# hadimsnj/SGRACEx1

Hardware: AMD Instinct MI355X
Metric: edges aggregated/sec, 2-layer GCN forward (higher is better)
Workload: dtype f16 (f32 accumulate); 1 GPU; s100m; nodes_per_gpu=4194304, edges_per_gpu=104193983, generator=uniform, f_in=1433, hidden=64, layer1=gemm_mode=0 sparse X, relu=1, layer2=gemm_mode=1 dense X, relu=0, exchange=none

## Files before the change

include/sgx.h:

```cpp
#ifndef SGX_H
#define SGX_H

#include <stddef.h>
#include <stdint.h>

#ifdef __cplusplus
extern "C" {
#endif

#define SGX_VERSION 110

typedef enum sgx_status {
    SGX_OK = 0,
    SGX_ERR_NULL = -1,
    SGX_ERR_SHAPE = -2,
    SGX_ERR_UNSUPPORTED = -3,
    SGX_ERR_WORKSPACE = -4,
    SGX_ERR_HIP = -5,
    SGX_ERR_CSR = -6,
    SGX_ERR_ALIGN = -7,
    SGX_ERR_SEEDS = -8,
    SGX_ERR_BLOCKS = -9
} sgx_status;

typedef enum sgx_dtype { SGX_F16 = 0, SGX_F32 = 1 } sgx_dtype;

typedef enum sgx_acc_mode { SGX_ACC_F32 = 0, SGX_ACC_REF_HALF = 1 } sgx_acc_mode;

typedef struct sgx_plan sgx_plan;

int sgx_plan_create(sgx_plan **plan, const int32_t *rowPtr, int n_rows, int n_feat_hint,
                    void *stream);
int sgx_plan_create_ex(sgx_plan **plan, const int32_t *rowPtr, int n_rows, int long_threshold, int chunk,
                       void *stream);
void sgx_plan_destroy(sgx_plan *plan);
int sgx_plan_long_rows(const sgx_plan *plan);
int sgx_plan_long_threshold(const sgx_plan *plan);
float sgx_plan_natural_utilization(const sgx_plan *plan);
int sgx_plan_reordered(const sgx_plan *plan);
int64_t sgx_plan_export(const sgx_plan *plan, int which, int32_t *dst, int64_t capacity, void *stream);
int sgx_xw_sparse_form(int dtype, int n_rows, int M_fea, int P, const void *W, int64_t ldw, const void *H, int64_t ldh,
                       const sgx_plan *plan);

#define SGX_QUANT_ADJ_DONE 1
#define SGX_QUANT_INT8 2
#define SGX_QUANT_INT8_AUTO 4
typedef struct sgx_quant {
    int32_t qbits;
    int32_t scale_fea;
    int32_t internal_bits;
    int32_t flags;
    float   inv_scale_fea;
    float   zero_fea;
    float   inv_scale_w;
    float   zero_w;
    float   inv_scale_adj;
    float   zero_adj;
    float   deq_factor;
    float   reserved;
    int64_t nnz_adj;
    int64_t nnz_fea;
} sgx_quant;

int sgx_fake_quantize(int is_signed, int qbits, float inv_scale, float zero, int64_t n, const float *x,
                      float *out, void *stream);
// ... 659 lines not shown
```

sgracex1_amd/csrc/layer.hip:

```cpp
#include "sgx_internal.h"

namespace {

struct Carve {
    size_t h_off, h_bytes;
    size_t w_off, w_bytes;
    size_t s_off, s_bytes;
    size_t g_off, g_bytes;
    size_t q_off, q_bytes;
    size_t qb, qx, qa, qt;
    size_t qw;
    int64_t ldc;
    size_t total;
};

bool repitch_x(const sgx_layer_desc *d)
{
    return sgx_ldh(d->dtype, d->M_fea) != d->M_fea && (int64_t)d->M_adj * d->M_fea >= (int64_t)1 << 22;
}

bool int8_form(const sgx_layer_desc *d)
{
    if (!d->quant || d->gemm_mode != 1 || d->quant->qbits > 8 || d->P_w > 256) return false;
    if (d->quant->flags & SGX_QUANT_INT8) return true;
// ... 194 lines not shown
        ep_d.out_scale = q->deq_factor;
    }

    int scores_ready = 0;
    if (d->gat_mode && !q && d->gemm_mode == 1 && d->acc_mode == SGX_ACC_F32 && attention &&
        sgx_gat_scores_fusable(d->dtype, d->P_w, d->gat_heads, d->plan_adj)) {
        const int heads = d->gat_heads < 1 ? 1 : d->gat_heads;
        float *gs = (float *)(ws + c.g_off);
        const sgx_gat_scratch lay = sgx_gat_scratch_layout(d->M_adj, d->P_w, heads, d->gat_fill_dead_rows, d->plan_adj);
        const bool direct = d->P_w / heads == 32;
        float *s1 = gs + (direct ? lay.s1 : lay.sp1), *s2 = gs + (direct ? lay.s2 : lay.sp2);
        rc = (direct || lay.has_partials)
                 ? sgx_xw_dense_scores(d->M_adj, d->M_fea, d->P_w, values_fea, d->M_fea, B, d->M_fea, H, ldh, attention, heads, s1, s2, s)
                 : SGX_ERR_UNSUPPORTED;
        if (rc == SGX_OK && !direct) rc = sgx_gat_scores_combine(gs, lay, d->M_adj, d->P_w, heads, s);
        if (rc == SGX_OK) scores_ready = 1;
        else if (rc != SGX_ERR_UNSUPPORTED) return rc;
    }
    if (scores_ready) {
        rc = SGX_OK;
    } else if (c.ldc) {
        rc = sgx_xw_dense_i8(q->qbits, d->M_adj, d->M_fea, d->P_w, (const int8_t *)values_fea, c.ldc, (const int8_t *)B, c.ldc,
                             q->scale_fea, q->internal_bits, (float *)H, ldh, ws + c.q_off + c.qw, s);
    } else if (d->gemm_mode == 0) {
        rc = sgx_transpose(d->dtype, d->P_w, d->M_fea, B, d->M_fea, W, ldh, s);
        if (rc != SGX_OK) return rc;
        rc = sgx_spmm_launch(d->dtype, d->acc_mode, d->spmm_block, 0, d->M_adj, d->M_fea, d->P_w, d->rowPtr_fea,
                             d->columnIndex_fea, values_fea, W, ldh, H, ldh, d->plan_fea, scratch, c.s_bytes, s, nullptr,
                             nullptr, 0, true, thread_count(d->fea_threads), ep_h);
    } else if (d->acc_mode == SGX_ACC_REF_HALF && thread_count(d->fea_threads) > 1) {
        if (d->dtype != SGX_F16) return SGX_ERR_UNSUPPORTED;
        if (ldh > d->P_w) SGX_HIP_CHECK(hipMemsetAsync(H, 0, (size_t)d->M_adj * ldh * sizeof(f16), s));
        rc = sgx_refhalf_dense(d->spmm_block, d->fea_threads, d->M_adj, d->M_fea, d->P_w, values_fea, d->M_fea, B, d->M_fea,
                               H, ldh, s);
    } else {
        rc = sgx_xw_dense_ep(d->dtype, d->acc_mode, d->spmm_block, d->M_adj, d->M_fea, d->P_w, values_fea, d->M_fea, B, d->M_fea,
                             H, ldh, s, ep_h);
    }
    if (rc != SGX_OK) return rc;

    if (d->ev_agg_begin) SGX_HIP_CHECK(hipEventRecord((hipEvent_t)d->ev_agg_begin, s));
    if (d->gat_mode) {
        if (!attention) return SGX_ERR_NULL;
        rc = sgx_gat_aggregate_ep(d->dtype, d->relu, d->gat_fill_dead_rows, d->N_adj, d->M_adj, d->P_w, d->gat_heads, d->alpha,
                                  d->rowPtr_adj, d->columnIndex_adj,
                                  values_adj, H, ldh, attention, d->D, d->P_w, (float *)d->E, (float *)d->S, d->plan_adj,
// ... 79 lines not shown
```

sgracex1_amd/csrc/sgx_internal.h:

```cpp
#pragma once
#include <hip/hip_runtime.h>
#include <stdint.h>
#include <stddef.h>

#include <atomic>
#include <type_traits>

#include "sgx.h"

#define SGX_HIP_CHECK(expr)                     \
    do {                                        \
        hipError_t _e = (expr);                 \
        if (_e != hipSuccess) return SGX_ERR_HIP; \
    } while (0)

#define SGX_LAUNCH_CHECK()                                   \
    do {                                                     \
        if (hipGetLastError() != hipSuccess) return SGX_ERR_HIP; \
    } while (0)

typedef _Float16 f16;

struct sgx_lds_optin {
    static constexpr int kDevices = 64;
    std::atomic<bool> done[kDevices];
};
template <typename Kernel>
int sgx_raise_dynamic_lds(Kernel kernel, sgx_lds_optin &optin, size_t bytes)
{
    int dev = 0;
    SGX_HIP_CHECK(hipGetDevice(&dev));
    const bool known = dev >= 0 && dev < sgx_lds_optin::kDevices;
    if (known && optin.done[dev].load(std::memory_order_acquire)) return SGX_OK;
    SGX_HIP_CHECK(hipFuncSetAttribute(reinterpret_cast<const void *>(kernel), hipFuncAttributeMaxDynamicSharedMemorySize, (int)bytes));
    if (known) optin.done[dev].store(true, std::memory_order_release);
    return SGX_OK;
}

struct sgx_tuning {
    bool gat_one_pass, gat_no_fused_scores;
    int gat_fused;
    int gat_scan;
    bool xw_no_wlds, xw_no_stationary_f32, xw_sparse_no_lds, xw_short_tiles, xw_no_lds;
    bool xtg_scalar, xtg_wave_tiles;
    bool spmm_no_short_tail;
    bool layer_no_fused_dense;
    int spmm_fused_blocks_per_cu;
    int spmm_cpl;
    int xw_sparse_lpr;
    int xw_sparse_streams;
    int plan_long_threshold;
    int plan_chunk;
    float plan_reorder_below;
};
const sgx_tuning &sgx_tune();

static inline size_t sgx_elem_size(int dtype) { return dtype == SGX_F16 ? 2 : 4; }
static inline size_t sgx_align_up(size_t x, size_t a) { return (x + a - 1) / a * a; }
static inline int sgx_next_pow2(int x) { int p = 1; while (p < x) p <<= 1; return p; }

struct sgx_plan {
    int n_rows;
    int64_t nnz;
    int long_threshold;
    int chunk;
    int n_long;
    int n_tasks;
    int32_t *long_row;
    int32_t *long_first;
    int32_t *task_row;
// ... 38 lines not shown
}

int sgx_refhalf_csr(int spmm_block, int threads, int relu, int n_rows, int n_cols, int n_feat, const int32_t *rowPtr, const int32_t *columnIndex,
                    const void *values, const void *table, int64_t ldt, void *out, int64_t ldo, hipStream_t s);
int sgx_refhalf_dense(int spmm_block, int threads, int n_rows, int M, int n_feat, const void *X, int64_t ldx, const void *Wt,
                      int64_t ldw, void *out, int64_t ldo, hipStream_t s);

int sgx_spmm_launch(int dtype, int acc_mode, int spmm_block, int relu, int n_rows, int n_cols, int n_feat,
                    const int32_t *rowPtr, const int32_t *columnIndex, const void *values,
                    const void *H, int64_t ldh, void *D, int64_t ldd,
                    const sgx_plan *plan, void *scratch, size_t scratch_bytes, hipStream_t stream,
                    const float *acc_in = nullptr, float *acc_out = nullptr, int64_t ld_acc = 0,
                    bool fea_stage = false, int ref_threads = 1, sgx_epilogue ep = sgx_no_epilogue());

bool sgx_spmm_table_big(int dtype, int n_cols, int64_t ldh, int n_feat);

bool sgx_spmm_dense_applicable(int n_cols, const void *X, const void *Wt, const void *D, const sgx_plan *plan);
int sgx_spmm_dense(int relu, int n_rows, int n_cols, const int32_t *rowPtr, const int32_t *columnIndex, const void *values,
                   const void *X, const void *Wt, void *D, hipStream_t stream);

bool sgx_xw_sparse_lds_applicable(int dtype, int n_rows, int m_fea, int n_feat, int64_t ldh, const sgx_plan *plan);
int sgx_xw_sparse_lds(int dtype, int n_rows, int m_fea, int n_feat, const int32_t *rowPtr, const int32_t *columnIndex,
                      const void *values, const void *W, int64_t ldw, void *H, int64_t ldh, const sgx_plan *plan,
                      sgx_epilogue ep, hipStream_t stream);

int sgx_repitch_rows(const void *src, int64_t src_pitch, void *dst, int64_t dst_pitch, int row_bytes, int64_t n_rows,
                     hipStream_t stream);
struct sgx_xw_form {
    int kind, a, b, blocks, vec, wgs_per_cu;
    int64_t waves;
};
bool sgx_xw_dense_wlds_form(int n_rows, int M, int P, const void *X, int64_t ldx, const void *Wt, int64_t ldw, const void *H,
                            int64_t ldh, sgx_xw_form *form);
bool sgx_xw_dense_wlds_f32_form(int n_rows, int M, int P, const void *Wt, int64_t ldw, const void *H, int64_t ldh, int h_aligned,
                                sgx_xw_form *form);
int sgx_xw_dense_wlds(int n_rows, int M, int P, const void *X, int64_t ldx, const void *Wt, int64_t ldw, void *H, int64_t ldh,
                      int relu, hipStream_t stream);
int sgx_xw_dense_wlds_f32(int n_rows, int M, int P, const void *X, int64_t ldx, const void *Wt, int64_t ldw, void *H, int64_t ldh,
                          int h_aligned, sgx_epilogue ep, int relu, hipStream_t stream);
int sgx_xw_dense_ep(int dtype, int acc_mode, int spmm_block, int n_rows, int M_fea, int P, const void *X, int64_t ldx,
                    const void *Wt, int64_t ldw, void *H, int64_t ldh, hipStream_t stream, sgx_epilogue ep, int relu = 0);
int sgx_gat_aggregate_ep(int dtype, int relu, int fill_dead_rows, int n_rows, int n_cols, int n_feat, int n_heads, float alpha,
                         const int32_t *rowPtr, const int32_t *columnIndex, const void *values, const void *Wh, int64_t ldh,
                         const void *attention, void *D, int64_t ldd, float *E, float *S, const sgx_plan *plan,
                         float *s_scratch, hipStream_t stream, float out_scale, const float *ext_fill = nullptr, int ext_n = 0,
                         int scores_ready = 0);

// ... 88 lines not shown
```

sgracex1_amd/csrc/spmm_csr.hip:

```cpp
#include "sgx_device.h"

#ifndef SGX_SPMM_MINWAVES
#define SGX_SPMM_MINWAVES 1
#endif
#ifndef SGX_SPMM_NT_STORE
#define SGX_SPMM_NT_STORE 0
#endif
#include <stdlib.h>

#ifndef SGX_SPMM_ADJ_STYLE
#define SGX_SPMM_ADJ_STYLE 0
#endif
#ifndef SGX_SPMM_FEA_STYLE
#define SGX_SPMM_FEA_STYLE 1
#endif
#ifndef SGX_SPMM_PIECES
#define SGX_SPMM_PIECES 1
#endif
#ifndef SGX_SPMM_BLOCKS_PER_CU
#define SGX_SPMM_BLOCKS_PER_CU 512
#endif

namespace {

// ... 295 lines not shown

template <typename T, int VEC, int LPR, int CPL, bool BIG>
__global__ __launch_bounds__(kBlock, SGX_SPMM_MINWAVES) void spmm_short_tail_kernel(SGX_SPMM_PARAMS)
{
    spmm_body<T, VEC, LPR, CPL, BIG, SGX_SPMM_ADJ_STYLE, true>(SGX_SPMM_ARGS);
}

template <typename T, int VEC, int LPR, int CPL, bool BIG>
__global__ __launch_bounds__(kBlock, SGX_SPMM_MINWAVES) void xw_sparse_kernel(SGX_SPMM_PARAMS)
{
    spmm_body<T, VEC, LPR, CPL, BIG, SGX_SPMM_FEA_STYLE, false>(SGX_SPMM_ARGS);
}

typedef _Float16 f16x8 __attribute__((ext_vector_type(8)));
typedef f16x8 f16x8_u __attribute__((aligned(2)));
typedef float f32x4 __attribute__((ext_vector_type(4)));

constexpr int kDenseF = 64;
constexpr int kDenseTile = 16;
constexpr int kDensePitch = kDenseF + 8;
#ifndef SGX_SPMM_DENSE_BLOCKS_PER_CU
#define SGX_SPMM_DENSE_BLOCKS_PER_CU 256
#endif

__device__ __forceinline__ void wave_lds_sync()
{
    __builtin_amdgcn_fence(__ATOMIC_RELEASE, "wavefront");
    __builtin_amdgcn_wave_barrier();
    __builtin_amdgcn_fence(__ATOMIC_ACQUIRE, "wavefront");
}

__global__ __launch_bounds__(kBlock, SGX_SPMM_MINWAVES) void spmm_dense_f16_kernel(
    int n_rows, const int32_t *__restrict__ rowptr, const int32_t *__restrict__ col, const f16 *__restrict__ val,
    const f16 *__restrict__ X, unsigned x_bytes, const f16 *__restrict__ Wt, f16 *__restrict__ D, int relu)
{
    constexpr int VEC = 8, LPR = 8, RPW = 64 / LPR, KS = kDenseF / 32, NT = kDenseF / 16;
    __shared__ __attribute__((aligned(16))) f16x8 sW[KS][NT][64];
    __shared__ __attribute__((aligned(16))) f16 sZ[kBlock / 64][kDenseTile * kDensePitch];
    const int lane = threadIdx.x & 63;
    const int sub = lane % LPR, grp = lane / LPR;
    const int l15 = lane & 15, lq = lane >> 4;

    for (int i = threadIdx.x; i < KS * NT * 64; i += kBlock) {
        const int ln = i & 63, nt = (i >> 6) % NT, s = i / (64 * NT);
        const int n = (nt / 2) * 32 + 8 * ((ln & 15) / 4) + 4 * (nt % 2) + (ln & 15) % 4;
        sW[s][nt][ln] = *reinterpret_cast<const f16x8_u *>(Wt + n * kDenseF + s * 32 + 8 * (ln >> 4));
    }
    __syncthreads();

    const __amdgpu_buffer_rsrc_t rsrc = __builtin_amdgcn_make_buffer_rsrc(const_cast<f16 *>(X), 0, x_bytes, 0x00020000);
    const unsigned chunk_off[1] = {(unsigned)(sub * VEC) * (unsigned)sizeof(f16)};
    f16 *slab = sZ[threadIdx.x >> 6];
// ... 28 lines not shown
#pragma unroll
            for (int nt = 0; nt < NT; ++nt) d[nt] = __builtin_amdgcn_mfma_f32_16x16x32_f16(sW[s][nt][lane], b, d[nt], 0, 0, 0);
        }
        wave_lds_sync();
#pragma unroll
        for (int q = 0; q < NT / 2; ++q) {
            f16x8 o;
#pragma unroll
            for (int j = 0; j < 4; ++j) {
                const f16 lo = (f16)d[2 * q][j], hi = (f16)d[2 * q + 1][j];
                o[j] = (!relu || lo > (f16)0) ? lo : (f16)0;
                o[4 + j] = (!relu || hi > (f16)0) ? hi : (f16)0;
            }
            *reinterpret_cast<f16x8 *>(slab + l15 * kDensePitch + q * 32 + 8 * lq) = o;
        }
        wave_lds_sync();
#pragma unroll
        for (int h = 0; h < kDenseTile / RPW; ++h) {
            const int64_t r = r0 + h * RPW + grp;
            const u32x4 v = *reinterpret_cast<const u32x4 *>(slab + (h * RPW + grp) * kDensePitch + sub * VEC);
            if (r < n_rows) *reinterpret_cast<Elem<f16>::vec16_u *>(D + r * kDenseF + sub * VEC) = v;
        }
        wave_lds_sync();
    }
}

template <typename T>
__global__ __launch_bounds__(kBlock) void spmm_split_finalize_kernel(
    int n_long, int n_feat, const int32_t *__restrict__ long_row, const int32_t *__restrict__ long_first,
    const float *__restrict__ partial, int ldp, T *__restrict__ D, int64_t ldd, int relu,
    const float *__restrict__ acc_in, float *__restrict__ acc_out, int64_t ld_acc, sgx_epilogue ep)
{
    const int64_t gid = (int64_t)blockIdx.x * kBlock + threadIdx.x;
    const int64_t total = (int64_t)n_long * n_feat;
    if (gid >= total) return;
    const int l = (int)(gid / n_feat), j = (int)(gid % n_feat);
    const int64_t row = long_row[l];
    float s = acc_in ? acc_in[row * ld_acc + j] : 0.0f;
    const int t_end = long_first[l + 1];
    int t = long_first[l];
    for (; t + 8 <= t_end; t += 8) {
        float v[8];
#pragma unroll
        for (int u = 0; u < 8; ++u) v[u] = partial[(int64_t)(t + u) * ldp + j];
#pragma unroll
        for (int u = 0; u < 8; ++u) s += v[u];
// ... 117 lines not shown
}

bool sgx_spmm_table_big(int dtype, int n_cols, int64_t ldh, int n_feat)
{
    const size_t es = sgx_elem_size(dtype);
    return (unsigned long long)n_cols * (unsigned long long)ldh * es > kOOBRow || (unsigned long long)n_feat * es > kMaxRowBytes;
}

bool sgx_spmm_dense_applicable(int n_cols, const void *X, const void *Wt, const void *D, const sgx_plan *plan)
{
    if (plan && (plan->n_tasks > 0 || plan->row_order)) return false;
    if (sgx_spmm_table_big(SGX_F16, n_cols, kDenseF, kDenseF)) return false;
    return (uintptr_t)X % 4 == 0 && (uintptr_t)Wt % 2 == 0 && (uintptr_t)D % 2 == 0;
}

int sgx_spmm_dense(int relu, int n_rows, int n_cols, const int32_t *rowPtr, const int32_t *columnIndex, const void *values,
                   const void *X, const void *Wt, void *D, hipStream_t stream)
{
    if (n_rows < 0 || n_cols < 0) return SGX_ERR_SHAPE;
    if (n_rows == 0) return SGX_OK;
    if (!rowPtr || !Wt || !D) return SGX_ERR_NULL;
    if (n_cols > 0 && (!X || !columnIndex || !values)) return SGX_ERR_NULL;
    if (!sgx_spmm_dense_applicable(n_cols, X, Wt, D, nullptr)) return SGX_ERR_UNSUPPORTED;
    const int64_t rows_per_block = (int64_t)kDenseTile * (kBlock / 64);
    int64_t blocks = ((int64_t)n_rows + rows_per_block - 1) / rows_per_block;
    const int per_cu = sgx_tune().spmm_fused_blocks_per_cu > 0 ? sgx_tune().spmm_fused_blocks_per_cu : SGX_SPMM_DENSE_BLOCKS_PER_CU;
    if (blocks > (int64_t)256 * per_cu) blocks = (int64_t)256 * per_cu;
    hipLaunchKernelGGL(spmm_dense_f16_kernel, dim3((unsigned)blocks), dim3(kBlock), 0, stream, n_rows, rowPtr, columnIndex,
                       (const f16 *)values, (const f16 *)X, (unsigned)((size_t)n_cols * kDenseF * sizeof(f16)), (const f16 *)Wt,
                       (f16 *)D, relu);
    SGX_LAUNCH_CHECK();
    return SGX_OK;
}

int sgx_spmm_launch(int dtype, int acc_mode, int spmm_block, int relu, int n_rows, int n_cols, int n_feat,
                    const int32_t *rowPtr, const int32_t *columnIndex, const void *values,
                    const void *H, int64_t ldh, void *D, int64_t ldd,
                    const sgx_plan *plan, void *scratch, size_t scratch_bytes, hipStream_t stream,
                    const float *acc_in, float *acc_out, int64_t ld_acc, bool fea_stage, int ref_threads, sgx_epilogue ep)
{
    (void)spmm_block;
    if (n_rows < 0 || n_cols < 0 || n_feat < 1 || ldh < n_feat) return SGX_ERR_SHAPE;
    if (n_rows == 0) return SGX_OK;
    if (!rowPtr || (!D && !acc_out)) return SGX_ERR_NULL;
    if (D && ldd < n_feat) return SGX_ERR_SHAPE;
    if ((acc_in || acc_out) && (ld_acc < n_feat || acc_mode != SGX_ACC_F32)) return SGX_ERR_SHAPE;
    if (dtype != SGX_F16 && dtype != SGX_F32) return SGX_ERR_UNSUPPORTED;
    if (acc_mode == SGX_ACC_REF_HALF) {
        if (dtype != SGX_F16) return SGX_ERR_UNSUPPORTED;
        if (n_cols > 0 && (!H || !columnIndex || !values)) return SGX_ERR_NULL;
        return sgx_refhalf_csr(spmm_block, ref_threads, relu, n_rows, n_cols, n_feat, rowPtr, columnIndex, values, H, ldh, D, ldd, stream);
    }
    if (acc_mode != SGX_ACC_F32) return SGX_ERR_UNSUPPORTED;
    if (plan && plan->n_rows != n_rows) return SGX_ERR_SHAPE;
    const size_t es = sgx_elem_size(dtype);
// ... 54 lines not shown
```

sgracex1_amd/csrc/util_kernels.hip:

```cpp
#include "sgx_internal.h"

#include <stdlib.h>

namespace {

constexpr int kBlock = 256;

template <typename T>
__global__ __launch_bounds__(kBlock) void transpose_kernel(int rows, int cols, const T *__restrict__ in, int64_t ldi,
                                                           T *__restrict__ out, int64_t ldo)
{
    __shared__ T tile[32][33];
    const int tx = threadIdx.x & 31, ty = threadIdx.x >> 5;
    const int r0 = blockIdx.y * 32, c0 = blockIdx.x * 32;
    for (int i = ty; i < 32; i += 8) {
        const int r = r0 + i, c = c0 + tx;
        tile[i][tx] = (r < rows && c < cols) ? in[(int64_t)r * ldi + c] : (T)0;
    }
    __syncthreads();
    for (int i = ty; i < 32; i += 8) {
        const int c = c0 + i, r = r0 + tx;
        if (c < cols && r < ldo) out[(int64_t)c * ldo + r] = (r < rows) ? tile[tx][i] : (T)0;
    }
}
// ... 237 lines not shown

namespace {
sgx_tuning g_tuning;
bool g_tuning_loaded = false;
void load_tuning()
{
    sgx_tuning t{};
    auto flag = [](const char *name) { return getenv(name) != nullptr; };
    auto num = [](const char *name) { const char *v = getenv(name); return v ? atoi(v) : 0; };
    t.gat_one_pass = flag("SGX_GAT_ONE_PASS");
    t.gat_no_fused_scores = flag("SGX_GAT_NO_FUSED_SCORES");
    { const char *v = getenv("SGX_GAT_SCAN"); t.gat_scan = v ? atoi(v) : 1; }
    { const char *v = getenv("SGX_GAT_FUSED"); t.gat_fused = v ? atoi(v) : 1; }
    t.xw_no_wlds = flag("SGX_XW_NO_WLDS");
    t.xw_no_stationary_f32 = flag("SGX_XW_NO_STATIONARY_F32");
    t.xw_sparse_no_lds = flag("SGX_XW_SPARSE_NO_LDS");
    t.xw_short_tiles = flag("SGX_XW_SHORT_TILES");
    t.xw_no_lds = flag("SGX_XW_NO_LDS");
    t.xtg_scalar = flag("SGX_XTG_SCALAR");
    t.xtg_wave_tiles = flag("SGX_XTG_WAVE_TILES");
    t.spmm_no_short_tail = flag("SGX_SPMM_NO_SHORT_TAIL");
    t.layer_no_fused_dense = flag("SGX_LAYER_NO_FUSED_DENSE");
    t.spmm_fused_blocks_per_cu = num("SGX_SPMM_FUSED_BLOCKS_PER_CU");
    t.spmm_cpl = num("SGX_SPMM_CPL");
    t.xw_sparse_lpr = num("SGX_XW_SPARSE_LPR");
    t.xw_sparse_streams = num("SGX_XW_SPARSE_STREAMS");
    t.plan_long_threshold = num("SGX_PLAN_LONG_THRESHOLD");
    t.plan_chunk = num("SGX_PLAN_CHUNK");
    const char *rb = getenv("SGX_PLAN_REORDER_BELOW");
    t.plan_reorder_below = rb ? (float)atof(rb) : -1.0f;
    g_tuning = t;
    g_tuning_loaded = true;
}
}

const sgx_tuning &sgx_tune()
{
    if (!g_tuning_loaded) load_tuning();
    return g_tuning;
}

extern "C" void sgx_reload_env(void) { load_tuning(); }
```

sgracex1_amd/csrc/xw_sparse_lds.hip:

```cpp
#include "sgx_device.h"

#include <stdlib.h>
#include <type_traits>

namespace {

constexpr int kWaves = 16;
constexpr int kThreads = kWaves * 64;
#ifndef SGX_XW_LDS_DEPTH
#define SGX_XW_LDS_DEPTH 8
#endif
#ifndef SGX_XW_LDS_SKIP_UNUSED
#define SGX_XW_LDS_SKIP_UNUSED 1
#endif
#ifndef SGX_XW_LDS_PAIRS
#define SGX_XW_LDS_PAIRS 0
#endif
constexpr unsigned kFarOOB = 0xFFFF0000u;
constexpr int kDepth = SGX_XW_LDS_DEPTH;
constexpr size_t kLdsBudget = 160 * 1024;

template <int EPS, int TT> __device__ __forceinline__ unsigned step_bcast(unsigned x)
{
    if constexpr (EPS == 1) return x;
    else if constexpr (EPS == 4)
        return (unsigned)__builtin_amdgcn_mov_dpp((int)x, TT | (TT << 2) | (TT << 4) | (TT << 6), 0xF, 0xF, true);
    else
        return (unsigned)__builtin_amdgcn_mov_dpp((int)x, TT | (TT << 2) | ((2 + TT) << 4) | ((2 + TT) << 6), 0xF, 0xF, true);
}

template <typename T, int VEC, int LPR, bool FULL>
__global__ __launch_bounds__(kThreads) void xw_sparse_lds_kernel(
    int n_rows, int n_feat, int m_fea, const int32_t *__restrict__ rowptr, const int32_t *__restrict__ col,
    const T *__restrict__ val, const T *__restrict__ W, int64_t ldw, int w_vec, T *__restrict__ H, int64_t ldh,
    int n_split, unsigned nnz_bytes_col, const uint8_t *__restrict__ win_order, sgx_epilogue ep)
{
    extern __shared__ __attribute__((aligned(16))) unsigned char lds[];
    constexpr int CP = LPR * VEC;
    constexpr unsigned ROWB = LPR * 16;
    constexpr int RPW = 64 / LPR;
    constexpr int SUBS = LPR;
    constexpr int EPS = LPR >= 4 ? 4 : LPR;
    constexpr int D = kDepth;

    const int xcd = blockIdx.x & 7, q = blockIdx.x >> 3;
    const int streams_per_xcd = (int)(gridDim.x >> 3) / n_split;
    if (q >= streams_per_xcd * n_split) return;
    const int split = q % n_split;
    const int stream = (q / n_split) * 8 + xcd;
    const int n_streams = streams_per_xcd * 8;
    const int c_base = split * CP;

    if (w_vec) {
        constexpr int kFill = 6;
        const int total = (m_fea + 1) * LPR;
        const __amdgpu_buffer_rsrc_t w_rsrc = __builtin_amdgcn_make_buffer_rsrc(
            const_cast<T *>(W), 0, (unsigned)(((int64_t)(m_fea - 1) * ldw + ldw) * (int64_t)sizeof(T)), 0x00020000);
        for (int i0 = threadIdx.x; i0 < total; i0 += kThreads * kFill) {
            u32x4 v[kFill];
#pragma unroll
            for (int f = 0; f < kFill; ++f) {
                const int i = i0 + kThreads * f;
                const int r = i / LPR, c0 = c_base + (i % LPR) * VEC;
                const bool in = i < total && r < m_fea && c0 + VEC <= ldw;
                v[f] = __builtin_amdgcn_raw_buffer_load_b128(w_rsrc, in ? (unsigned)(((int64_t)r * ldw + c0) * (int64_t)sizeof(T)) : kOOB, 0, 0);
            }
#pragma unroll
            for (int f = 0; f < kFill; ++f) {
                const int i = i0 + kThreads * f;
                if (i < total) *reinterpret_cast<u32x4 *>(lds + (size_t)i * 16) = v[f];
            }
        }
    } else {
        for (int i = threadIdx.x; i < (m_fea + 1) * LPR; i += kThreads) {
            const int r = i / LPR, c0 = c_base + (i % LPR) * VEC;
            union { u32x4 v; T e[VEC]; } u;
// ... 313 lines not shown
    const int64_t es = dtype == SGX_F16 ? 2 : 4;
    const int cp = f.lpr * (int)(16 / es);
    f.lds_bytes = (size_t)(m_fea + 1) * f.lpr * 16;
    f.n_split = (n_feat + cp - 1) / cp;
    f.full = n_feat % cp == 0 && ((uintptr_t)H % 16 == 0) && ((ldh * es) % 16 == 0);
    f.w_vec = ((uintptr_t)W % 16 == 0) && ((ldw * es) % 16 == 0);
    f.wgs_per_cu = f.lds_bytes * 2 <= kLdsBudget ? 2 : 1;
    int grid = device_cus() / 8 * 8 * f.wgs_per_cu;
    const int64_t tiles = ((int64_t)n_work + 64 * kWaves - 1) / (64 * kWaves);
    const int64_t want = (tiles + 7) / 8 * 8 * f.n_split;
    if (want < grid) grid = (int)want;
    if (sgx_tune().xw_sparse_streams > 0) {
        const int streams = sgx_tune().xw_sparse_streams / 8 * 8;
        const int cap = (streams < 8 ? 8 : streams) * f.n_split;
        if (cap < grid) grid = cap;
    }
    if (grid < 8 * f.n_split) grid = 8 * f.n_split;
    f.grid = grid;
    return f;
}

template <typename T, int VEC, int LPR, bool FULL>
int launch_lds_impl(const LdsForm &f, int n_work, int n_feat, int m_fea, const int32_t *rowptr, const int32_t *col, const void *val,
                    const void *W, int64_t ldw, void *H, int64_t ldh, int64_t nnz, const uint8_t *win_order, sgx_epilogue ep,
                    hipStream_t stream)
{
    auto kernel = xw_sparse_lds_kernel<T, VEC, LPR, FULL>;
    static sgx_lds_optin optin;
    const int rc = sgx_raise_dynamic_lds(kernel, optin, kLdsBudget);
    if (rc != SGX_OK) return rc;
    hipLaunchKernelGGL(kernel, dim3(f.grid), dim3(kThreads), f.lds_bytes, stream, n_work, n_feat, m_fea, rowptr, col,
                       (const T *)val, (const T *)W, ldw, f.w_vec, (T *)H, ldh, f.n_split, (unsigned)(nnz * 4), win_order, ep);
    SGX_LAUNCH_CHECK();
    return SGX_OK;
}

template <typename T, int VEC, int LPR>
int launch_lds(const LdsForm &f, int n_work, int n_feat, int m_fea, const int32_t *rowptr, const int32_t *col, const void *val,
               const void *W, int64_t ldw, void *H, int64_t ldh, int64_t nnz, const uint8_t *win_order, sgx_epilogue ep,
               hipStream_t stream)
{
    return f.full ? launch_lds_impl<T, VEC, LPR, true>(f, n_work, n_feat, m_fea, rowptr, col, val, W, ldw, H, ldh, nnz, win_order, ep, stream)
                  : launch_lds_impl<T, VEC, LPR, false>(f, n_work, n_feat, m_fea, rowptr, col, val, W, ldw, H, ldh, nnz, win_order, ep, stream);
}

}

bool sgx_xw_sparse_lds_applicable(int dtype, int n_rows, int m_fea, int n_feat, int64_t ldh, const sgx_plan *plan)
{
    if (sgx_tune().xw_sparse_no_lds) return false;
    if (!plan || !plan->win_order || plan->n_tasks > 0 || plan->nnz < ((int64_t)1 << 20) || plan->nnz >= ((int64_t)1 << 30) - 65536 || n_rows < 4096)
        return false;
    if ((unsigned long long)n_rows * (unsigned long long)ldh * (dtype == SGX_F16 ? 2ull : 4ull) >= 0xFFF00000ull)
        return false;
    const int lpr = choose_lpr(dtype, m_fea, n_feat);
    if (lpr < 1) return false;
    const int per16 = dtype == SGX_F16 ? 8 : 4;
    const int n_split = (n_feat + lpr * per16 - 1) / (lpr * per16);
    return n_split <= 4;
}

int sgx_xw_sparse_lds(int dtype, int n_rows, int m_fea, int n_feat, const int32_t *rowPtr, const int32_t *columnIndex,
                      const void *values, const void *W, int64_t ldw, void *H, int64_t ldh, const sgx_plan *plan,
                      sgx_epilogue ep, hipStream_t stream)
{
    const int n_work = n_rows;
    const LdsForm f = lds_form(dtype, n_work, m_fea, n_feat, W, ldw, H, ldh);
#define SGX_LDS_CASE(L)                                                                                                     \
    case L:                                                                                                                 \
        return dtype == SGX_F16 ? launch_lds<f16, 8, L>(f, n_work, n_feat, m_fea, rowPtr, columnIndex, values, W, ldw, H,   \
                                                        ldh, plan->nnz, plan->win_order, ep, stream)                        \
                                : launch_lds<float, 4, L>(f, n_work, n_feat, m_fea, rowPtr, columnIndex, values, W, ldw, H, \
                                                          ldh, plan->nnz, plan->win_order, ep, stream);
    switch (f.lpr) {
        SGX_LDS_CASE(2)
        SGX_LDS_CASE(4)
        SGX_LDS_CASE(8)
        SGX_LDS_CASE(16)
    default: return SGX_ERR_UNSUPPORTED;
    }
#undef SGX_LDS_CASE
}

extern "C" int sgx_xw_sparse_form(int dtype, int n_rows, int M_fea, int P, const void *W, int64_t ldw, const void *H, int64_t ldh,
                                  const sgx_plan *plan)
{
    if ((dtype != SGX_F16 && dtype != SGX_F32) || n_rows < 1 || M_fea < 0 || P < 1 || ldw < P || ldh < P) return 0;
    if (plan && plan->n_rows != n_rows) return 0;
    if (sgx_spmm_table_big(dtype, M_fea, ldw, P)) return 0;
    if (!sgx_xw_sparse_lds_applicable(dtype, n_rows, M_fea, P, ldh, plan)) return 0;
    const LdsForm f = lds_form(dtype, n_rows, M_fea, P, W, ldw, H, ldh);
    if (f.lpr < 2) return 0;
    return f.lpr | f.n_split << 8 | f.full << 16 | f.w_vec << 17 | f.wgs_per_cu << 18 | f.streams() << 20;
}
```

sgracex1_amd/ops.py:

```python
import collections
import ctypes

import numpy as np
import torch

from . import _lib
from ._lib import (SGX_ACC_F32, SGX_ACC_REF_HALF, SGX_F16, SGX_F32, SGX_ORDER_AGGREGATE_FIRST, SGX_ORDER_REFERENCE,
                   LayerDesc, check, lib)

_DTYPES = {torch.float16: SGX_F16, torch.float32: SGX_F32}


def dtype_code(dtype):
    try:
        return _DTYPES[dtype]
    except KeyError:
        raise TypeError(f"sgx supports float16 and float32 element types, got {dtype}") from None


def _dev(t, name):
    if not isinstance(t, torch.Tensor) or not t.is_cuda:
        raise ValueError(f"{name} must be a tensor on the GPU (got {type(t).__name__}"
                         f"{'' if not isinstance(t, torch.Tensor) else ' on ' + str(t.device)})")
    if not t.is_contiguous():
# ... 287 lines not shown
    scratch = _workspace(H.device, sbytes) if sbytes else None
    check(lib.sgx_spmm_csr(code, acc_mode, spmm_block, int(bool(relu)), adj.n_rows, H.shape[0], n_feat,
                           _ptr(adj.rowptr), _ptr(adj.col), _ptr(adj.val), _ptr(H), H.stride(0),
                           _ptr(out), out.stride(0), plan.handle if plan is not None else None,
                           _ptr(scratch), sbytes, _stream()), "sgx_spmm_csr")
    return out


def xw_sparse(X, W, out=None, use_plan=True):
    _dev2d(W, "W")
    if X.val.dtype != W.dtype:
        raise TypeError("feature values and W must share one element type (MM.h:129-139)")
    if W.shape[0] < X.n_cols:
        raise ValueError(f"W has {W.shape[0]} rows, X refers to {X.n_cols} columns")
    P = W.shape[1]
    W = _gatherable(W, P, X.nnz)
    out = _out(out, X.n_rows, P, W.dtype, W.device)
    plan = X.plan if (use_plan and X.wants_plan) else None
    sbytes = lib.sgx_spmm_scratch_bytes(plan.handle, P) if plan is not None else 0
    scratch = _workspace(W.device, sbytes) if sbytes else None
    check(lib.sgx_xw_sparse(dtype_code(W.dtype), SGX_ACC_F32, 1, X.n_rows, X.n_cols, P, _ptr(X.rowptr), _ptr(X.col),
                            _ptr(X.val), _ptr(W), W.stride(0), _ptr(out), out.stride(0),
                            plan.handle if plan is not None else None, _ptr(scratch), sbytes, _stream()), "sgx_xw_sparse")
    return out


XwSparseForm = collections.namedtuple("XwSparseForm", "lpr n_split full w_vec wgs_per_cu streams")


def xw_sparse_form(X, W, out=None, use_plan=True):
    _dev2d(W, "W")
    P = W.shape[1]
    if _gatherable_copies(W, P, X.nnz):
        w_ptr, ldw = None, table_pitch(P, W.element_size())
    else:
        w_ptr, ldw = _ptr(W), W.stride(0)
    if out is None:
        h_ptr, ldh = None, P
    else:
        out = _out(out, X.n_rows, P, W.dtype, W.device)
        h_ptr, ldh = _ptr(out), out.stride(0)
    plan = X.plan if (use_plan and X.wants_plan) else None
    word = lib.sgx_xw_sparse_form(dtype_code(W.dtype), X.n_rows, X.n_cols, P, w_ptr, ldw, h_ptr, ldh,
                                  plan.handle if plan is not None else None)
    if word == 0:
        return None
# ... 1892 lines not shown
```

Baseline: 44.47 billion edges/s.

## Read transposed W directly in sparse XW LDS kernel and add warp-specialized dense spmm

Layer 1 with sparse features now routes through the LDS-resident sparse XW kernel, which loads W by strided element gathers from its original layout instead of running a separate transpose kernel followed by a generic sparse-times-dense launch. Separately, a producer/consumer dense spmm kernel is added in which gather wavefronts fill double-buffered LDS slabs and one wavefront runs the MFMA epilogue, coordinated with workgroup-scope flags. The dense variant is disabled by default and selected by environment variables. The strided W fill issues many small loads per block, and the spin-wait handoff risks idle waves.

New measurement: 44.45 billion edges/s. About the same (-0.0%).

```diff
diff --git a/include/sgx.h b/include/sgx.h
--- a/include/sgx.h
+++ b/include/sgx.h
@@ -41,6 +41,10 @@
 int64_t sgx_plan_export(const sgx_plan *plan, int which, int32_t *dst, int64_t capacity, void *stream);
 int sgx_xw_sparse_form(int dtype, int n_rows, int M_fea, int P, const void *W, int64_t ldw, const void *H, int64_t ldh,
                        const sgx_plan *plan);
+int sgx_spmm_dense_gather_waves(void);
+int sgx_xw_sparse_wt(int dtype, int acc_mode, int n_rows, int M_fea, int P, const int32_t *rowPtr,
+                     const int32_t *columnIndex, const void *values, const void *Wt, int64_t ldwt, void *H, int64_t ldh,
+                     const sgx_plan *plan, void *stream);
 
 #define SGX_QUANT_ADJ_DONE 1
 #define SGX_QUANT_INT8 2
diff --git a/sgracex1_amd/csrc/layer.hip b/sgracex1_amd/csrc/layer.hip
--- a/sgracex1_amd/csrc/layer.hip
+++ b/sgracex1_amd/csrc/layer.hip
@@ -240,6 +240,11 @@
     } else if (c.ldc) {
         rc = sgx_xw_dense_i8(q->qbits, d->M_adj, d->M_fea, d->P_w, (const int8_t *)values_fea, c.ldc, (const int8_t *)B, c.ldc,
                              q->scale_fea, q->internal_bits, (float *)H, ldh, ws + c.q_off + c.qw, s);
+    } else if (d->gemm_mode == 0 &&
+               sgx_xw_sparse_wt_applicable(d->dtype, d->acc_mode, d->M_adj, d->M_fea, d->P_w, d->M_fea, ldh, ldh, d->plan_fea)) {
+        if (!d->columnIndex_fea || !values_fea) return SGX_ERR_NULL;
+        rc = sgx_xw_sparse_lds(d->dtype, d->M_adj, d->M_fea, d->P_w, d->rowPtr_fea, d->columnIndex_fea, values_fea, B, d->M_fea, H,
+                               ldh, d->plan_fea, ep_h, s, true);
     } else if (d->gemm_mode == 0) {
         rc = sgx_transpose(d->dtype, d->P_w, d->M_fea, B, d->M_fea, W, ldh, s);
         if (rc != SGX_OK) return rc;
diff --git a/sgracex1_amd/csrc/sgx_internal.h b/sgracex1_amd/csrc/sgx_internal.h
--- a/sgracex1_amd/csrc/sgx_internal.h
+++ b/sgracex1_amd/csrc/sgx_internal.h
@@ -46,6 +46,8 @@
     bool spmm_no_short_tail;
     bool layer_no_fused_dense;
     int spmm_fused_blocks_per_cu;
+    int spmm_dense_epilogue_waves;
+    int spmm_dense_gather_waves;
     int spmm_cpl;
     int xw_sparse_lpr;
     int xw_sparse_streams;
@@ -130,7 +132,9 @@
 bool sgx_xw_sparse_lds_applicable(int dtype, int n_rows, int m_fea, int n_feat, int64_t ldh, const sgx_plan *plan);
 int sgx_xw_sparse_lds(int dtype, int n_rows, int m_fea, int n_feat, const int32_t *rowPtr, const int32_t *columnIndex,
                       const void *values, const void *W, int64_t ldw, void *H, int64_t ldh, const sgx_plan *plan,
-                      sgx_epilogue ep, hipStream_t stream);
+                      sgx_epilogue ep, hipStream_t stream, bool w_transposed = false);
+bool sgx_xw_sparse_wt_applicable(int dtype, int acc_mode, int n_rows, int m_fea, int n_feat, int64_t ldwt, int64_t ldw_rowmajor,
+                                 int64_t ldh, const sgx_plan *plan);
 
 int sgx_repitch_rows(const void *src, int64_t src_pitch, void *dst, int64_t dst_pitch, int row_bytes, int64_t n_rows,
                      hipStream_t stream);
diff --git a/sgracex1_amd/csrc/spmm_csr.hip b/sgracex1_amd/csrc/spmm_csr.hip
--- a/sgracex1_amd/csrc/spmm_csr.hip
+++ b/sgracex1_amd/csrc/spmm_csr.hip
@@ -341,12 +341,94 @@
 #ifndef SGX_SPMM_DENSE_BLOCKS_PER_CU
 #define SGX_SPMM_DENSE_BLOCKS_PER_CU 256
 #endif
+#ifndef SGX_SPMM_DENSE_EPILOGUE_WAVES
+#define SGX_SPMM_DENSE_EPILOGUE_WAVES 0
+#endif
+#ifndef SGX_SPMM_DENSE_GATHER_WAVES
+#define SGX_SPMM_DENSE_GATHER_WAVES 7
+#endif
 
 __device__ __forceinline__ void wave_lds_sync()
 {
     __builtin_amdgcn_fence(__ATOMIC_RELEASE, "wavefront");
     __builtin_amdgcn_wave_barrier();
     __builtin_amdgcn_fence(__ATOMIC_ACQUIRE, "wavefront");
+}
+
+constexpr int kDenseKS = kDenseF / 32, kDenseNT = kDenseF / 16;
+typedef f16x8 dense_w_frags[kDenseKS][kDenseNT][64];
+
+template <int THREADS> __device__ __forceinline__ void dense_fill_w(dense_w_frags &sW, const f16 *__restrict__ Wt)
+{
+    constexpr int KS = kDenseKS, NT = kDenseNT;
+    for (int i = threadIdx.x; i < KS * NT * 64; i += THREADS) {
+        const int ln = i & 63, nt = (i >> 6) % NT, s = i / (64 * NT);
+        const int n = (nt / 2) * 32 + 8 * ((ln & 15) / 4) + 4 * (nt % 2) + (ln & 15) % 4;
+        sW[s][nt][ln] = *reinterpret_cast<const f16x8_u *>(Wt + n * kDenseF + s * 32 + 8 * (ln >> 4));
+    }
+}
+
+__device__ __forceinline__ void dense_gather_tile(f16 *slab, int64_t r0, int n_rows, const int32_t *__restrict__ rowptr,
+                                                  const int32_t *__restrict__ col, const f16 *__restrict__ val,
+                                                  const __amdgpu_buffer_rsrc_t rsrc, const f16 *__restrict__ X, int lane)
+{
+    constexpr int VEC = 8, LPR = 8, RPW = 64 / LPR;
+    const int sub = lane % LPR, grp = lane / LPR;
+    const unsigned chunk_off[1] = {(unsigned)(sub * VEC) * (unsigned)sizeof(f16)};
+#pragma unroll 1
+    for (int h = 0; h < kDenseTile / RPW; ++h) {
+        const int64_t r = r0 + h * RPW + grp;
+        int e0 = 0, e1 = 0;
+        if (r < n_rows) {
+            e0 = rowptr[r];
+            e1 = rowptr[r + 1];
+        }
+        float acc[VEC];
+#pragma unroll
+        for (int i = 0; i < VEC; ++i) acc[i] = 0.0f;
+        accumulate_edges<f16, VEC, LPR, 1, false, SGX_SPMM_ADJ_STYLE>(acc, e0, e1, LPR, sub, col, val, rsrc, X,
+                                                                      kDenseF * (unsigned)sizeof(f16), chunk_off);
+        f16x8 z;
+#pragma unroll
+        for (int i = 0; i < VEC; ++i) z[i] = (f16)acc[i];
+        *reinterpret_cast<f16x8 *>(slab + (h * RPW + grp) * kDensePitch + sub * VEC) = z;
+    }
+}
+
+__device__ __forceinline__ void dense_tile_epilogue(f16 *slab, const dense_w_frags &sW, int64_t r0, int n_rows,
+                                                    f16 *__restrict__ D, int relu, int lane)
+{
+    constexpr int VEC = 8, LPR = 8, RPW = 64 / LPR, KS = kDenseKS, NT = kDenseNT;
+    const int sub = lane % LPR, grp = lane / LPR;
+    const int l15 = lane & 15, lq = lane >> 4;
+    f32x4 d[NT];
+#pragma unroll
+    for (int nt = 0; nt < NT; ++nt) d[nt] = (f32x4){0, 0, 0, 0};
+#pragma unroll
+    for (int s = 0; s < KS; ++s) {
+        const f16x8 b = *reinterpret_cast<const f16x8 *>(slab + l15 * kDensePitch + s * 32 + 8 * lq);
+#pragma unroll
+        for (int nt = 0; nt < NT; ++nt) d[nt] = __builtin_amdgcn_mfma_f32_16x16x32_f16(sW[s][nt][lane], b, d[nt], 0, 0, 0);
+    }
+    wave_lds_sync();
+#pragma unroll
+    for (int q = 0; q < NT / 2; ++q) {
+        f16x8 o;
+#pragma unroll
+        for (int j = 0; j < 4; ++j) {
+            const f16 lo = (f16)d[2 * q][j], hi = (f16)d[2 * q + 1][j];
+            o[j] = (!relu || lo > (f16)0) ? lo : (f16)0;
+            o[4 + j] = (!relu || hi > (f16)0) ? hi : (f16)0;
+        }
+        *reinterpret_cast<f16x8 *>(slab + l15 * kDensePitch + q * 32 + 8 * lq) = o;
+    }
+    wave_lds_sync();
+#pragma unroll
+    for (int h = 0; h < kDenseTile / RPW; ++h) {
+        const int64_t r = r0 + h * RPW + grp;
+        const u32x4 v = *reinterpret_cast<const u32x4 *>(slab + (h * RPW + grp) * kDensePitch + sub * VEC);
+        if (r < n_rows) *reinterpret_cast<Elem<f16>::vec16_u *>(D + r * kDenseF + sub * VEC) = v;
+    }
 }
 
 __global__ __launch_bounds__(kBlock, SGX_SPMM_MINWAVES) void spmm_dense_f16_kernel(
@@ -421,6 +503,72 @@
             if (r < n_rows) *reinterpret_cast<Elem<f16>::vec16_u *>(D + r * kDenseF + sub * VEC) = v;
         }
         wave_lds_sync();
+    }
+}
+
+constexpr int kDenseRing = 2;
+constexpr unsigned kSlabDone = 0xFFFFFFFFu;
+
+__device__ __forceinline__ unsigned slab_state(const unsigned *word)
+{
+    return (unsigned)__builtin_amdgcn_readfirstlane((int)__hip_atomic_load(word, __ATOMIC_ACQUIRE, __HIP_MEMORY_SCOPE_WORKGROUP));
+}
+__device__ __forceinline__ void slab_publish(unsigned *word, unsigned state, int lane)
+{
+    __builtin_amdgcn_fence(__ATOMIC_RELEASE, "workgroup");
+    if (lane == 0) __hip_atomic_store(word, state, __ATOMIC_RELAXED, __HIP_MEMORY_SCOPE_WORKGROUP);
+}
+
+template <int G>
+__global__ __launch_bounds__((G + 1) * 64, SGX_SPMM_MINWAVES) void spmm_dense_f16_ew_kernel(
+    int n_rows, const int32_t *__restrict__ rowptr, const int32_t *__restrict__ col, const f16 *__restrict__ val,
+    const f16 *__restrict__ X, unsigned x_bytes, const f16 *__restrict__ Wt, f16 *__restrict__ D, int relu)
+{
+    static_assert(G >= 1 && G < 32 && kDenseRing == 2, "one bit per gather wavefront: seen-done and ring position");
+    __shared__ __attribute__((aligned(16))) dense_w_frags sW;
+    __shared__ __attribute__((aligned(16))) f16 sZ[G][kDenseRing][kDenseTile * kDensePitch];
+    __shared__ unsigned sState[G][kDenseRing];
+    const int lane = threadIdx.x & 63;
+    const int wid = __builtin_amdgcn_readfirstlane((int)(threadIdx.x >> 6));
+    dense_fill_w<(G + 1) * 64>(sW, Wt);
+    if (threadIdx.x < G * kDenseRing) (&sState[0][0])[threadIdx.x] = 0u;
+    __syncthreads();
+
+    if (wid < G) {
+        const __amdgpu_buffer_rsrc_t rsrc = __builtin_amdgcn_make_buffer_rsrc(const_cast<f16 *>(X), 0, x_bytes, 0x00020000);
+        const int64_t wave = (int64_t)blockIdx.x * G + wid;
+        const int64_t n_waves = (int64_t)gridDim.x * G;
+        int slot = 0;
+        for (int64_t r0 = wave * kDenseTile; r0 < n_rows; r0 += n_waves * kDenseTile) {
+            while (slab_state(&sState[wid][slot]) != 0u) __builtin_amdgcn_s_sleep(8);
+            dense_gather_tile(sZ[wid][slot], r0, n_rows, rowptr, col, val, rsrc, X, lane);
+            slab_publish(&sState[wid][slot], (unsigned)r0 + 1u, lane);
+            slot ^= 1;
+        }
+        while (slab_state(&sState[wid][slot]) != 0u) __builtin_amdgcn_s_sleep(8);
+        slab_publish(&sState[wid][slot], kSlabDone, lane);
+        return;
+    }
+
+    unsigned done = 0u, pos = 0u;
+    while (done != (1u << G) - 1u) {
+        bool idle = true;
+#pragma unroll 1
+        for (int g = 0; g < G; ++g) {
+            if (done >> g & 1u) continue;
+            const int slot = (int)(pos >> g & 1u);
+            const unsigned state = slab_state(&sState[g][slot]);
+            if (state == 0u) continue;
+            idle = false;
+            if (state == kSlabDone) {
+                done |= 1u << g;
+                continue;
+            }
+            dense_tile_epilogue(sZ[g][slot], sW, (int64_t)(state - 1u), n_rows, D, relu, lane);
+            slab_publish(&sState[g][slot], 0u, lane);
+            pos ^= 1u << g;
+        }
+        if (idle) __builtin_amdgcn_s_sleep(16);
     }
 }
 
@@ -584,15 +732,31 @@
     if (!rowPtr || !Wt || !D) return SGX_ERR_NULL;
     if (n_cols > 0 && (!X || !columnIndex || !values)) return SGX_ERR_NULL;
     if (!sgx_spmm_dense_applicable(n_cols, X, Wt, D, nullptr)) return SGX_ERR_UNSUPPORTED;
-    const int64_t rows_per_block = (int64_t)kDenseTile * (kBlock / 64);
+    const int gather_waves = sgx_spmm_dense_gather_waves();
+    const int64_t rows_per_block = (int64_t)kDenseTile * (gather_waves ? gather_waves : kBlock / 64);
     int64_t blocks = ((int64_t)n_rows + rows_per_block - 1) / rows_per_block;
     const int per_cu = sgx_tune().spmm_fused_blocks_per_cu > 0 ? sgx_tune().spmm_fused_blocks_per_cu : SGX_SPMM_DENSE_BLOCKS_PER_CU;
     if (blocks > (int64_t)256 * per_cu) blocks = (int64_t)256 * per_cu;
-    hipLaunchKernelGGL(spmm_dense_f16_kernel, dim3((unsigned)blocks), dim3(kBlock), 0, stream, n_rows, rowPtr, columnIndex,
-                       (const f16 *)values, (const f16 *)X, (unsigned)((size_t)n_cols * kDenseF * sizeof(f16)), (const f16 *)Wt,
-                       (f16 *)D, relu);
+    const unsigned x_bytes = (unsigned)((size_t)n_cols * kDenseF * sizeof(f16));
+#define SGX_DENSE_LAUNCH(KERNEL, WAVES)                                                                                     \
+    hipLaunchKernelGGL(KERNEL, dim3((unsigned)blocks), dim3((WAVES) * 64), 0, stream, n_rows, rowPtr, columnIndex,         \
+                       (const f16 *)values, (const f16 *)X, x_bytes, (const f16 *)Wt, (f16 *)D, relu)
+    switch (gather_waves) {
+    case 0: SGX_DENSE_LAUNCH(spmm_dense_f16_kernel, kBlock / 64); break;
+    case 4: SGX_DENSE_LAUNCH(spmm_dense_f16_ew_kernel<4>, 5); break;
+    default: SGX_DENSE_LAUNCH(spmm_dense_f16_ew_kernel<7>, 8); break;
+    }
+#undef SGX_DENSE_LAUNCH
     SGX_LAUNCH_CHECK();
     return SGX_OK;
+}
+
+extern "C" int sgx_spmm_dense_gather_waves(void)
+{
+    const int ew = sgx_tune().spmm_dense_epilogue_waves >= 0 ? sgx_tune().spmm_dense_epilogue_waves : SGX_SPMM_DENSE_EPILOGUE_WAVES;
+    if (ew <= 0) return 0;
+    const int g = sgx_tune().spmm_dense_gather_waves > 0 ? sgx_tune().spmm_dense_gather_waves : SGX_SPMM_DENSE_GATHER_WAVES;
+    return g == 4 ? 4 : 7;
 }
 
 int sgx_spmm_launch(int dtype, int acc_mode, int spmm_block, int relu, int n_rows, int n_cols, int n_feat,
diff --git a/sgracex1_amd/csrc/util_kernels.hip b/sgracex1_amd/csrc/util_kernels.hip
--- a/sgracex1_amd/csrc/util_kernels.hip
+++ b/sgracex1_amd/csrc/util_kernels.hip
@@ -283,6 +283,8 @@
     t.spmm_no_short_tail = flag("SGX_SPMM_NO_SHORT_TAIL");
     t.layer_no_fused_dense = flag("SGX_LAYER_NO_FUSED_DENSE");
     t.spmm_fused_blocks_per_cu = num("SGX_SPMM_FUSED_BLOCKS_PER_CU");
+    { const char *v = getenv("SGX_SPMM_DENSE_EPILOGUE_WAVES"); t.spmm_dense_epilogue_waves = v ? atoi(v) : -1; }
+    t.spmm_dense_gather_waves = num("SGX_SPMM_DENSE_GATHER_WAVES");
     t.spmm_cpl = num("SGX_SPMM_CPL");
     t.xw_sparse_lpr = num("SGX_XW_SPARSE_LPR");
     t.xw_sparse_streams = num("SGX_XW_SPARSE_STREAMS");
diff --git a/sgracex1_amd/csrc/xw_sparse_lds.hip b/sgracex1_amd/csrc/xw_sparse_lds.hip
--- a/sgracex1_amd/csrc/xw_sparse_lds.hip
+++ b/sgracex1_amd/csrc/xw_sparse_lds.hip
@@ -19,6 +19,7 @@
 constexpr unsigned kFarOOB = 0xFFFF0000u;
 constexpr int kDepth = SGX_XW_LDS_DEPTH;
 constexpr size_t kLdsBudget = 160 * 1024;
+constexpr int kFillElem = 0, kFillVec = 1, kFillWt = 2;
 
 template <int EPS, int TT> __device__ __forceinline__ unsigned step_bcast(unsigned x)
 {
@@ -32,7 +33,7 @@
 template <typename T, int VEC, int LPR, bool FULL>
 __global__ __launch_bounds__(kThreads) void xw_sparse_lds_kernel(
     int n_rows, int n_feat, int m_fea, const int32_t *__restrict__ rowptr, const int32_t *__restrict__ col,
-    const T *__restrict__ val, const T *__restrict__ W, int64_t ldw, int w_vec, T *__restrict__ H, int64_t ldh,
+    const T *__restrict__ val, const T *__restrict__ W, int64_t ldw, int w_fill, T *__restrict__ H, int64_t ldh,
     int n_split, unsigned nnz_bytes_col, const uint8_t *__restrict__ win_order, sgx_epilogue ep)
 {
     extern __shared__ __attribute__((aligned(16))) unsigned char lds[];
@@ -51,7 +52,36 @@
     const int n_streams = streams_per_xcd * 8;
     const int c_base = split * CP;
 
-    if (w_vec) {
+    if (w_fill == kFillWt) {
+        constexpr int kFill = 6;
+        const int total = (m_fea + 1) * LPR;
+        const __amdgpu_buffer_rsrc_t w_rsrc = __builtin_amdgcn_make_buffer_rsrc(
+            const_cast<T *>(W), 0, (unsigned)(((int64_t)(n_feat - 1) * ldw + m_fea) * (int64_t)sizeof(T)), 0x00020000);
+        const unsigned col_pitch = (unsigned)ldw * (unsigned)sizeof(T);
+        for (int i0 = threadIdx.x; i0 < total; i0 += kThreads * kFill) {
+            union { u32x4 v; T e[VEC]; } u[kFill];
+#pragma unroll
+            for (int f = 0; f < kFill; ++f) {
+                const int i = i0 + kThreads * f;
+                const int r = i / LPR, c0 = c_base + (i % LPR) * VEC;
+                const bool row_in = i < total && r < m_fea;
+                const unsigned base = (unsigned)c0 * col_pitch + (unsigned)r * (unsigned)sizeof(T);
+#pragma unroll
+                for (int j = 0; j < VEC; ++j) {
+                    const unsigned off = (row_in && c0 + j < n_feat) ? base + (unsigned)j * col_pitch : kOOB;
+                    if constexpr (sizeof(T) == 2)
+                        u[f].e[j] = __builtin_bit_cast(T, (unsigned short)__builtin_amdgcn_raw_buffer_load_b16(w_rsrc, off, 0, 0));
+                    else
+                        u[f].e[j] = __builtin_bit_cast(T, __builtin_amdgcn_raw_buffer_load_b32(w_rsrc, off, 0, 0));
+                }
+            }
+#pragma unroll
+            for (int f = 0; f < kFill; ++f) {
+                const int i = i0 + kThreads * f;
+                if (i < total) *reinterpret_cast<u32x4 *>(lds + (size_t)i * 16) = u[f].v;
+            }
+        }
+    } else if (w_fill == kFillVec) {
         constexpr int kFill = 6;
         const int total = (m_fea + 1) * LPR;
         const __amdgpu_buffer_rsrc_t w_rsrc = __builtin_amdgcn_make_buffer_rsrc(
@@ -411,26 +441,26 @@
 
 template <typename T, int VEC, int LPR, bool FULL>
 int launch_lds_impl(const LdsForm &f, int n_work, int n_feat, int m_fea, const int32_t *rowptr, const int32_t *col, const void *val,
-                    const void *W, int64_t ldw, void *H, int64_t ldh, int64_t nnz, const uint8_t *win_order, sgx_epilogue ep,
-                    hipStream_t stream)
+                    const void *W, int64_t ldw, int w_fill, void *H, int64_t ldh, int64_t nnz, const uint8_t *win_order,
+                    sgx_epilogue ep, hipStream_t stream)
 {
     auto kernel = xw_sparse_lds_kernel<T, VEC, LPR, FULL>;
     static sgx_lds_optin optin;
     const int rc = sgx_raise_dynamic_lds(kernel, optin, kLdsBudget);
     if (rc != SGX_OK) return rc;
     hipLaunchKernelGGL(kernel, dim3(f.grid), dim3(kThreads), f.lds_bytes, stream, n_work, n_feat, m_fea, rowptr, col,
-                       (const T *)val, (const T *)W, ldw, f.w_vec, (T *)H, ldh, f.n_split, (unsigned)(nnz * 4), win_order, ep);
+                       (const T *)val, (const T *)W, ldw, w_fill, (T *)H, ldh, f.n_split, (unsigned)(nnz * 4), win_order, ep);
     SGX_LAUNCH_CHECK();
     return SGX_OK;
 }
 
 template <typename T, int VEC, int LPR>
 int launch_lds(const LdsForm &f, int n_work, int n_feat, int m_fea, const int32_t *rowptr, const int32_t *col, const void *val,
-               const void *W, int64_t ldw, void *H, int64_t ldh, int64_t nnz, const uint8_t *win_order, sgx_epilogue ep,
-               hipStream_t stream)
-{
-    return f.full ? launch_lds_impl<T, VEC, LPR, true>(f, n_work, n_feat, m_fea, rowptr, col, val, W, ldw, H, ldh, nnz, win_order, ep, stream)
-                  : launch_lds_impl<T, VEC, LPR, false>(f, n_work, n_feat, m_fea, rowptr, col, val, W, ldw, H, ldh, nnz, win_order, ep, stream);
+               const void *W, int64_t ldw, int w_fill, void *H, int64_t ldh, int64_t nnz, const uint8_t *win_order,
+               sgx_epilogue ep, hipStream_t stream)
+{
+    return f.full ? launch_lds_impl<T, VEC, LPR, true>(f, n_work, n_feat, m_fea, rowptr, col, val, W, ldw, w_fill, H, ldh, nnz, win_order, ep, stream)
+                  : launch_lds_impl<T, VEC, LPR, false>(f, n_work, n_feat, m_fea, rowptr, col, val, W, ldw, w_fill, H, ldh, nnz, win_order, ep, stream);
 }
 
 }
@@ -451,16 +481,17 @@
 
 int sgx_xw_sparse_lds(int dtype, int n_rows, int m_fea, int n_feat, const int32_t *rowPtr, const int32_t *columnIndex,
                       const void *values, const void *W, int64_t ldw, void *H, int64_t ldh, const sgx_plan *plan,
-                      sgx_epilogue ep, hipStream_t stream)
+                      sgx_epilogue ep, hipStream_t stream, bool w_transposed)
 {
     const int n_work = n_rows;
-    const LdsForm f = lds_form(dtype, n_work, m_fea, n_feat, W, ldw, H, ldh);
+    const LdsForm f = lds_form(dtype, n_work, m_fea, n_feat, w_transposed ? nullptr : W, w_transposed ? n_feat : ldw, H, ldh);
+    const int w_fill = w_transposed ? kFillWt : (f.w_vec ? kFillVec : kFillElem);
 #define SGX_LDS_CASE(L)                                                                                                     \
     case L:                                                                                                                 \
-        return dtype == SGX_F16 ? launch_lds<f16, 8, L>(f, n_work, n_feat, m_fea, rowPtr, columnIndex, values, W, ldw, H,   \
-                                                        ldh, plan->nnz, plan->win_order, ep, stream)                        \
-                                : launch_lds<float, 4, L>(f, n_work, n_feat, m_fea, rowPtr, columnIndex, values, W, ldw, H, \
-                                                          ldh, plan->nnz, plan->win_order, ep, stream);
+        return dtype == SGX_F16 ? launch_lds<f16, 8, L>(f, n_work, n_feat, m_fea, rowPtr, columnIndex, values, W, ldw,      \
+                                                        w_fill, H, ldh, plan->nnz, plan->win_order, ep, stream)             \
+                                : launch_lds<float, 4, L>(f, n_work, n_feat, m_fea, rowPtr, columnIndex, values, W, ldw,    \
+                                                          w_fill, H, ldh, plan->nnz, plan->win_order, ep, stream);
     switch (f.lpr) {
         SGX_LDS_CASE(2)
         SGX_LDS_CASE(4)
@@ -471,6 +502,29 @@
 #undef SGX_LDS_CASE
 }
 
+bool sgx_xw_sparse_wt_applicable(int dtype, int acc_mode, int n_rows, int m_fea, int n_feat, int64_t ldwt, int64_t ldw_rowmajor,
+                                 int64_t ldh, const sgx_plan *plan)
+{
+    if ((dtype != SGX_F16 && dtype != SGX_F32) || acc_mode != SGX_ACC_F32) return false;
+    if (n_rows < 1 || m_fea < 1 || n_feat < 1 || ldwt < m_fea || ldw_rowmajor < n_feat || ldh < n_feat) return false;
+    if (plan && plan->n_rows != n_rows) return false;
+    if (sgx_spmm_table_big(dtype, m_fea, ldw_rowmajor, n_feat)) return false;
+    if ((unsigned long long)n_feat * (unsigned long long)ldwt * (dtype == SGX_F16 ? 2ull : 4ull) >= 0xFFF00000ull) return false;
+    return sgx_xw_sparse_lds_applicable(dtype, n_rows, m_fea, n_feat, ldh, plan);
+}
+
+extern "C" int sgx_xw_sparse_wt(int dtype, int acc_mode, int n_rows, int M_fea, int P, const int32_t *rowPtr,
+                                const int32_t *columnIndex, const void *values, const void *Wt, int64_t ldwt, void *H,
+                                int64_t ldh, const sgx_plan *plan, void *stream)
+{
+    if (n_rows < 0 || M_fea < 0 || P < 1 || ldwt < M_fea || ldh < P) return SGX_ERR_SHAPE;
+    if (n_rows == 0) return SGX_OK;
+    if (!rowPtr || !columnIndex || !values || !Wt || !H) return SGX_ERR_NULL;
+    if (!sgx_xw_sparse_wt_applicable(dtype, acc_mode, n_rows, M_fea, P, ldwt, P, ldh, plan)) return SGX_ERR_UNSUPPORTED;
+    return sgx_xw_sparse_lds(dtype, n_rows, M_fea, P, rowPtr, columnIndex, values, Wt, ldwt, H, ldh, plan, sgx_no_epilogue(),
+                             (hipStream_t)stream, true);
+}
+
 extern "C" int sgx_xw_sparse_form(int dtype, int n_rows, int M_fea, int P, const void *W, int64_t ldw, const void *H, int64_t ldh,
                                   const sgx_plan *plan)
 {
diff --git a/sgracex1_amd/ops.py b/sgracex1_amd/ops.py
--- a/sgracex1_amd/ops.py
+++ b/sgracex1_amd/ops.py
@@ -333,6 +333,21 @@
     check(lib.sgx_xw_sparse(dtype_code(W.dtype), SGX_ACC_F32, 1, X.n_rows, X.n_cols, P, _ptr(X.rowptr), _ptr(X.col),
                             _ptr(X.val), _ptr(W), W.stride(0), _ptr(out), out.stride(0),
                             plan.handle if plan is not None else None, _ptr(scratch), sbytes, _stream()), "sgx_xw_sparse")
+    return out
+
+
+def xw_sparse_wt(X, Wt, out=None):
+    _dev2d(Wt, "Wt")
+    if X.val.dtype != Wt.dtype:
+        raise TypeError("feature values and Wt must share one element type (MM.h:129-139)")
+    if Wt.shape[1] < X.n_cols:
+        raise ValueError(f"Wt has {Wt.shape[1]} columns, X refers to {X.n_cols} columns")
+    P = Wt.shape[0]
+    out = _out(out, X.n_rows, P, Wt.dtype, Wt.device)
+    plan = X.plan if X.wants_plan else None
+    check(lib.sgx_xw_sparse_wt(dtype_code(Wt.dtype), SGX_ACC_F32, X.n_rows, X.n_cols, P, _ptr(X.rowptr), _ptr(X.col),
+                               _ptr(X.val), _ptr(Wt), Wt.stride(0), _ptr(out), out.stride(0),
+                               plan.handle if plan is not None else None, _stream()), "sgx_xw_sparse_wt")
     return out
 
 
```
